# arhix52/Strelka

Hardware: AMD Instinct MI355X
Metric: Mray/s (higher is better)
Workload: dtype f32; 1 GPU; kitchen stand-in (SURVEY 8d C3): 1724134 unique triangles, 2022 instances of 153 meshes, 4 rect + 1 distant light, 60/25/10/5 % diffuse/glossy/metal/glass; resolution=1920x1080, bounces=4, spp=64, tile=32, world_size=1, parallelism=single GPU, rays_per_frame=839862650

## Files before the change

strelka_amd/csrc/skh_kernels.h:

```cpp
#pragma once
#include "skh_bvh.h"
#include "skh_env.h"
#include "skh_emit.h"
#include "skh_blend.h"

namespace skh
{

struct DevInstance
{
    float w2o[12];
    int rootRef;
    uint32_t mask;
    uint32_t type;
    uint32_t pad;
};
struct HostInstance
{
    float o2w[12];
    uint32_t type, geom, material, light;
};

#define SKH_WORLD_CURVES 2
#define SKH_SEG_STRIDE 8
// ... 151 lines not shown
    unsigned long long wave[2][10];
    unsigned long long shade[8];
    unsigned int slowCount, slowPad;
    float slow[16][12];
    unsigned long long runHist[2][42], blockHist[2][42];
    unsigned long long cyc[2][10];
#endif
#ifdef SKH_TAIL_PROFILE
    unsigned long long launchT0[2], dryHist[2][64], exitHist[2][64], afterDryHist[2][64], dryLive[2][65], rayTicksAfterDry[2], waveTicksAfterDry[2];
#endif
};

SKH_DI uint32_t rank_below(unsigned long long mask)
{
    return __builtin_amdgcn_mbcnt_hi((uint32_t)(mask >> 32), __builtin_amdgcn_mbcnt_lo((uint32_t)mask, 0u));
}
SKH_DI uint32_t wave_max(uint32_t v)
{
#pragma unroll
    for (int off = 32; off >= 1; off >>= 1)
        v = max(v, (uint32_t)__shfl_xor(v, off));
    return v;
}

SKH_DI uint32_t wave_sum(uint32_t v)
{
#pragma unroll
    for (int off = 32; off >= 1; off >>= 1)
        v += __shfl_xor(v, off);
    return v;
}

#ifndef SKH_CURVE_MIN_WAVES
#define SKH_CURVE_MIN_WAVES 6
#endif
#ifndef SKH_WORLD_CURVE_ANYHIT_MIN_WAVES
#define SKH_WORLD_CURVE_ANYHIT_MIN_WAVES 6
#endif
#ifndef SKH_WORLD_CURVE_MIN_WAVES
#define SKH_WORLD_CURVE_MIN_WAVES 6
#endif
#ifndef SKH_ANYHIT_MIN_WAVES
#define SKH_ANYHIT_MIN_WAVES 7
#endif
#ifndef SKH_TRACE_MIN_WAVES
#define SKH_TRACE_MIN_WAVES 7
#endif
#ifndef SKH_MATERIALS_LDS
#define SKH_MATERIALS_LDS 64
#endif
#ifndef SKH_WORLD_ANYHIT_MIN_WAVES
#define SKH_WORLD_ANYHIT_MIN_WAVES 8
#endif
#ifndef SKH_WORLD_CLOSEST_MIN_WAVES
#define SKH_WORLD_CLOSEST_MIN_WAVES 8
#endif
#ifndef SKH_TRACE_ATTR
#define SKH_TRACE_ATTR
#endif
#ifndef SKH_TRI_COOP
#define SKH_TRI_COOP 1
#endif
#define SKH_FETCH_STRIDE 32
#define SKH_COUNT_STRIDE 32

SKH_DI uint32_t skh_opaque(uint32_t v)
{
    asm volatile("" : "+s"(v));
    return v;
}
struct LightBox
{
    float lo[3], hi[3];
};
#ifndef SKH_BEST_LDS
#define SKH_BEST_LDS 1
#endif
#ifndef SKH_SEGNODE
#define SKH_SEGNODE 0
#endif
#ifndef SKH_ANYHIT_FLAT_PUSH
#define SKH_ANYHIT_FLAT_PUSH 1
#endif
template <bool ANY_HIT, bool COUNT, bool CURVES, bool WORLD = false, bool SPLIT = false>
__global__ void __launch_bounds__(SKH_TRACE_BLOCK, CURVES ? (WORLD ? (ANY_HIT ? SKH_WORLD_CURVE_ANYHIT_MIN_WAVES : SKH_WORLD_CURVE_MIN_WAVES) : SKH_CURVE_MIN_WAVES) : (WORLD ? (ANY_HIT ? SKH_WORLD_ANYHIT_MIN_WAVES : SKH_WORLD_CLOSEST_MIN_WAVES) : (ANY_HIT ? SKH_ANYHIT_MIN_WAVES : SKH_TRACE_MIN_WAVES))) SKH_TRACE_ATTR
    k_trace(DevScene sc, RayQ rq, const uint32_t* __restrict__ countPtr, uint32_t* __restrict__ fetch ,
            uint32_t fetchArg ,
            HitQ hq, PathS ps, const float4* __restrict__ contrib , int* __restrict__ ovfBase,
            StatsDev* __restrict__ stats, LightBox lightBox , uint32_t fetchChunk )
{
    constexpr bool TRICOOP = SKH_TRI_COOP && WORLD && !CURVES;
    constexpr bool BESTLDS = CURVES && !ANY_HIT && SKH_BEST_LDS;
    static_assert(!SPLIT || (WORLD && !CURVES), "SPLIT: the world-only triangle builds");
    constexpr int NLDS0 = (TRICOOP || BESTLDS) ? SKH_STACK_LDS - 1 : SKH_STACK_LDS;
    constexpr int NLDST = (SPLIT && NLDS0 >= 11) ? NLDS0 - 7 : NLDS0;
    static_assert(NLDS0 - NLDST <= SKH_TAIL_EXTRA, "the overflow columns' extra slots hold the LDS entries the tail phase gives up");
    __shared__ int s_stack[NLDS0 * SKH_TRACE_BLOCK];
    __shared__ uint32_t s_famx[(SPLIT && NLDST == NLDS0) ? 7 * SKH_TRACE_BLOCK : 1];
    uint32_t* const s_fam = NLDST < NLDS0 ? reinterpret_cast<uint32_t*>(s_stack + NLDST * SKH_TRACE_BLOCK) : s_famx;
    __shared__ uint32_t s_best[BESTLDS ? 4 * SKH_TRACE_BLOCK : 1];
    __shared__ unsigned char s_tab[(TRICOOP || SPLIT) ? 128 : 1];
    const uint32_t fetchMin = fetchArg & 0xffu, curveMin = (fetchArg >> 8) & 0xffu, nodeBreak = (fetchArg >> 16) & 0xffu, leafMin = fetchArg >> 24;
    const uint32_t lane = threadIdx.x;
    uint32_t n = 0;
#pragma unroll
    for (uint32_t g = 0; g < SKH_SHARDS; ++g)
        n += countPtr[g * SKH_COUNT_STRIDE];
    if (n == 0)
        return;
    const uint32_t perGroup = rq.region;
    const uint32_t group = blockIdx.x & 7u;
    uint32_t tries = 0;
    bool exhausted = false;
    uint32_t resBase = 0, resLeft = 0;
    uint32_t fam = threadIdx.x;
#define SKH_FAM(k, l) s_fam[(k) * SKH_TRACE_BLOCK + (l)]
    int* lds = s_stack + lane;
#define SKH_OVF_SLOT(e) ((SKH_TAIL_PHASE && (e) < NLDS0) ? SKH_STACK_OVF + ((e) - NLDSP) : (e) - NLDS0)
#define SKH_OVF_AT(e) ovfBase[(size_t)(e) * ovfStride + (skh_opaque(blockIdx.x * SKH_TRACE_BLOCK) + threadIdx.x)]
    const uint32_t ovfStride = gridDim.x * SKH_TRACE_BLOCK;
    const uint32_t rayMask = CURVES ? (ANY_HIT ? 3u : 255u) : (ANY_HIT ? 1u : 253u);
    TraceCounters tc = { 0, 0, 0, 0 };
#ifdef SKH_LANE_PROFILE
    uint32_t wv[10] = { 0, 0, 0, 0, 0, 0, 0, 0, 0, 0 };
    uint32_t rayNodes = 0, rayTris = 0, rayInsts = 0;
    unsigned long long cy[7] = { 0, 0, 0, 0, 0, 0, 0 };
    const unsigned long long cyStart = __builtin_readcyclecounter();
    const unsigned long long rtStart = __builtin_amdgcn_s_memrealtime();
#define SKH_LP(...) __VA_ARGS__
#else
#define SKH_LP(...)
#endif
#ifdef SKH_TAIL_PROFILE
    if (threadIdx.x == 0)
        atomicMin(&stats->launchT0[ANY_HIT ? 1 : 0], (unsigned long long)__builtin_amdgcn_s_memrealtime());
    bool dryNoted = false;
    unsigned long long dryLast = 0, dryAt = 0, rayTicks = 0;
    uint32_t dryLiveLanes = 0;
#endif

    bool hasRay = false, pending = false;
    uint32_t pend = 0;
    uint32_t ridx = 0;
    v3 ow = mk3(0.0f), dw = mk3(0.0f), o = mk3(0.0f), d = mk3(0.0f), inv = mk3(0.0f);
    v3 invw = mk3(0.0f);
    float tmin = 0.0f;
    RayShear sh;
    sh.perm = 0;
    sh.Sx = sh.Sy = sh.Sz = 0.0f;
    const Node4* nodes = sc.tlasNodes;
    bool inBlas = false;
    uint32_t curInst = 0, curType = 0;
    int sp = 0, cur = SKH_REF_INVALID;
    HitRec best;
    best.t = 0.0f, best.inst = best.prim = 0xffffffffu, best.u = best.v = 0.0f, best.found = false;

#define SKH_BEST_INST() (BESTLDS ? s_best[lane] : best.inst)
#define SKH_BEST_PRIM() (BESTLDS ? s_best[SKH_TRACE_BLOCK + lane] : best.prim)
#define SKH_BEST_SET(INST, PRIM, U, V)                                                                \
    {                                                                                                 \
        if (BESTLDS)                                                                                  \
        {                                                                                             \
            s_best[lane] = (INST), s_best[SKH_TRACE_BLOCK + lane] = (PRIM);                           \
            s_best[2 * SKH_TRACE_BLOCK + lane] = __float_as_uint(U), s_best[3 * SKH_TRACE_BLOCK + lane] = __float_as_uint(V); \
        }                                                                                             \
        else                                                                                          \
            best.inst = (INST), best.prim = (PRIM), best.u = (U), best.v = (V);                       \
    }
#define SKH_HIDDEN_LIGHT(C) (ANY_HIT && __float_as_uint((C).w) != 0u)
#define SKH_PUSH(v)                                                  \
    {                                                                \
        if (sp < NLDSP)                                              \
            lds[sp * SKH_TRACE_BLOCK] = (v);                         \
        else if (sp < NLDS0 + SKH_STACK_OVF)                         \
            SKH_OVF_AT(SKH_OVF_SLOT(sp)) = (v);                      \
        else                                                         \
            *sc.overflowFlag = 1u;  \
        ++sp;                                                        \
    }
#define SKH_POP(dst)                                                 \
    {                                                                \
        --sp;                                                        \
        if (sp < NLDSP)                                              \
            dst = lds[sp * SKH_TRACE_BLOCK];                         \
        else if (sp < NLDS0 + SKH_STACK_OVF)                         \
            dst = SKH_OVF_AT(SKH_OVF_SLOT(sp));                      \
        else                                                         \
            dst = SKH_REF_INVALID;                                   \
    }

#define SKH_CYLINDER_TESTS(FIRST, COUNT, PEND)                                                                                   \
    for (uint32_t k_ = 0; k_ < (COUNT); ++k_)                                                                                    \
// ... 9 lines not shown
    }
#define SKH_TAKE_MARKER()                                                                                         \
    {                                                                                                             \
        const uint32_t k = (uint32_t)cur & 0xffffu;                                                               \
        const uint32_t xinst = sc.worldCurveInst[k];           \
        curInst = ((sc.worldCurveMerged >> k) & 1u) ? 0xffffffffu : xinst;  \
        if ((uint32_t)cur & SKH_REF_CURVEROOT_IDENT)                                                              \
        {                                                                                                         \
             \
             \
            const float ident[12] = { 1.0f, 0.0f, 0.0f, 0.0f, 0.0f, 1.0f, 0.0f, 0.0f, 0.0f, 0.0f, 1.0f, 0.0f };    \
            o = xform_point_rel(ident, o);                                                                        \
            d = xform_vector(ident, d);                                                                           \
        }                                                                                                         \
        else                                                                                                      \
        {                                                                                                         \
            const float4* ip = reinterpret_cast<const float4*>(sc.inst + xinst);                                  \
            const float4 i0 = ip[0], i1 = ip[1], i2 = ip[2];                                                      \
            const v3 wo = mk3(rq.plane(0)[ridx], rq.plane(1)[ridx], rq.plane(2)[ridx]);                           \
            const v3 wd = mk3(rq.plane(3)[ridx], rq.plane(4)[ridx], rq.plane(5)[ridx]);                           \
            const float m[12] = { i0.x, i0.y, i0.z, i0.w, i1.x, i1.y, i1.z, i1.w, i2.x, i2.y, i2.z, i2.w };       \
            o = xform_point_rel(m, wo);                                                                           \
            d = xform_vector(m, wd);                                                                              \
        }                                                                                                         \
        inv = rcp3(d);                                                                                            \
        curType = 2;                                                                                              \
        cur = sc.worldCurveRoot[k];                                                                               \
    }

    {
        constexpr int NLDSP = NLDS0;
        constexpr bool TRICOOPP = TRICOOP;
#define SKH_TAIL_PHASE 0
        for (;;)
        {
#include "skh_trace_body.inc"
        }
#undef SKH_TAIL_PHASE
    }
    if constexpr (SPLIT)
    {
        constexpr int NLDSP = NLDST;
#ifndef SKH_TAIL_TRICOOP
#define SKH_TAIL_TRICOOP 1
#endif
        constexpr bool TRICOOPP = TRICOOP && SKH_TAIL_TRICOOP;
        if (NLDST < NLDS0)
        {
            for (int e = NLDST; e < NLDS0; ++e)
                if (hasRay && e < sp)
                    SKH_OVF_AT(SKH_STACK_OVF + e - NLDST) = lds[e * SKH_TRACE_BLOCK];
            __builtin_amdgcn_fence(__ATOMIC_RELEASE, "wavefront");
            __builtin_amdgcn_wave_barrier();
            __builtin_amdgcn_fence(__ATOMIC_ACQUIRE, "wavefront");
        }
        if (hasRay)
        {
            fam = lane;
            SKH_FAM(0, lane) = __float_as_uint(best.t);
            SKH_FAM(1, lane) = __float_as_uint(best.t);
            SKH_FAM(2, lane) = best.found ? (ANY_HIT ? 0u : best.inst) : 0xffffffffu;
            if constexpr (!ANY_HIT)
                SKH_FAM(3, lane) = best.prim, SKH_FAM(4, lane) = __float_as_uint(best.u), SKH_FAM(5, lane) = __float_as_uint(best.v);
            SKH_FAM(6, lane) = 1u;
        }
        __builtin_amdgcn_fence(__ATOMIC_RELEASE, "wavefront");
        __builtin_amdgcn_wave_barrier();
        __builtin_amdgcn_fence(__ATOMIC_ACQUIRE, "wavefront");
#define SKH_TAIL_PHASE 1
        for (;;)
        {
#include "skh_trace_body.inc"
        }
#undef SKH_TAIL_PHASE
    }
#undef SKH_PUSH
#undef SKH_HIDDEN_LIGHT
#undef SKH_POP
#undef SKH_OVF_AT
#undef SKH_OVF_SLOT
#undef SKH_TAKE_MARKER
#undef SKH_CYLINDER_TESTS
#undef SKH_FAM
#ifdef SKH_TAIL_PROFILE
    if (lane == 0 && dryNoted)
    {
        const int A = ANY_HIT ? 1 : 0;
        const unsigned long long t0 = *(volatile unsigned long long*)&stats->launchT0[A], now = __builtin_amdgcn_s_memrealtime();
        atomicAdd(&stats->dryHist[A][min(63ull, (dryAt - t0) / 1600ull)], 1ull);
        atomicAdd(&stats->exitHist[A][min(63ull, (now - t0) / 1600ull)], 1ull);
        atomicAdd(&stats->afterDryHist[A][min(63ull, (now - dryAt) / 1600ull)], 1ull);
        atomicAdd(&stats->dryLive[A][dryLiveLanes], 1ull);
        atomicAdd(&stats->rayTicksAfterDry[A], rayTicks);
        atomicAdd(&stats->waveTicksAfterDry[A], now - dryAt);
    }
#endif
    if (COUNT)
    {
        const uint32_t a = wave_sum(tc.nodes), b = wave_sum(tc.prims), c2 = wave_sum(tc.segs), d2 = wave_sum(tc.insts);
#ifdef SKH_LANE_PROFILE
        cy[5] = __builtin_readcyclecounter() - cyStart;
        if (lane == 0)
        {
            atomicAdd(&stats->cyc[ANY_HIT ? 1 : 0][6], cy[5]);
            atomicAdd(&stats->cyc[ANY_HIT ? 1 : 0][7], __builtin_amdgcn_s_memrealtime() - rtStart);
        }
        for (int k = 0; k < 7; ++k)
        {
            uint32_t hi = wave_max((uint32_t)(cy[k] >> 8));
            if (lane == 0)
                atomicAdd(&stats->cyc[ANY_HIT ? 1 : 0][k == 6 ? 8 : k], (unsigned long long)hi << 8);
        }
#endif
        if (lane == 0)
        {
            atomicAdd(&stats->nodes[ANY_HIT ? 1 : 0], (unsigned long long)a);
            atomicAdd(&stats->prims[ANY_HIT ? 1 : 0], (unsigned long long)b);
            atomicAdd(&stats->segs[ANY_HIT ? 1 : 0], (unsigned long long)c2);
            atomicAdd(&stats->insts[ANY_HIT ? 1 : 0], (unsigned long long)d2);
#ifdef SKH_LANE_PROFILE
            for (int k = 0; k < 10; ++k)
                atomicAdd(&stats->wave[ANY_HIT ? 1 : 0][k], (unsigned long long)wv[k]);
#endif
        }
    }
#undef SKH_LP
}

__global__ void k_hair_consts(const Material* __restrict__ mats, uint32_t n, HairConst* __restrict__ out)
{
    const uint32_t i = blockIdx.x * blockDim.x + threadIdx.x;
    if (i < n)
        out[i] = hair_const(mats[i]);
}

SKH_DI bool slot_to_pixel(const FrameP& fp, const uint32_t* __restrict__ tileXY, uint32_t slot, uint32_t& px, uint32_t& py)
{
    const uint32_t tile = slot >> (2 * fp.tileShift);
    const uint32_t m = slot & ((1u << (2 * fp.tileShift)) - 1u);
    px = tileXY[2 * tile] + compact1by1(m);
    py = tileXY[2 * tile + 1] + compact1by1(m >> 1);
    return px < fp.width && py < fp.height;
}

#define SKH_COMPACT_MAX_WAVES 8
SKH_DI uint32_t block_compact(bool emit, uint32_t* counter, uint32_t* s_wave )
{
    const uint32_t lane = threadIdx.x & 63u, wave = threadIdx.x >> 6, nw = blockDim.x >> 6;
    const unsigned long long m = __ballot(emit);
    if (lane == 0)
        s_wave[wave] = (uint32_t)__popcll(m);
    __syncthreads();
    if (threadIdx.x == 0)
    {
        uint32_t tot = 0;
        for (uint32_t w = 0; w < nw; ++w)
        {
            const uint32_t cnt = s_wave[w];
            s_wave[w] = tot;
            tot += cnt;
        }
        s_wave[SKH_COMPACT_MAX_WAVES] = tot ? atomicAdd(counter, tot) : 0u;
    }
    __syncthreads();
    const uint32_t r = s_wave[SKH_COMPACT_MAX_WAVES] + s_wave[wave] + rank_below(m);
    __syncthreads();
// ... 1044 lines not shown
```

strelka_amd/csrc/skh_shade_body.inc:

```
    const uint32_t numPick = (ENV ? sc.numLights + (env.nee ? 1u : 0u) : sc.numLights) + (EMIT ? (emit.nee ? 1u : 0u) : 0u);
    __shared__ uint32_t s_wave[2 * (SKH_COMPACT_MAX_WAVES + 1)];
    __shared__ uint32_t s_sobol[SKH_SOBOL_LUT_WORDS];
#if SKH_MATERIALS_LDS
    __shared__ float4 s_mat[SKH_MATERIALS_LDS * 4];
#endif
    const uint32_t shard = blockIdx.x & (SKH_SHARDS - 1u), lb = blockIdx.x / SKH_SHARDS;
    const uint32_t n = countPtr[shard * SKH_COUNT_STRIDE];
    if (lb * blockDim.x >= n)
        return;
    const uint32_t il = lb * blockDim.x + threadIdx.x;
    const uint32_t i = shard * rq.region + il;
#ifdef SKH_LANE_PROFILE
    unsigned long long spc[8] = { 0, 0, 0, 0, 0, 0, 0, 0 }, spT = __builtin_readcyclecounter();
#define SKH_SP(k)                                                    \
    {                                                                \
        const unsigned long long t_ = __builtin_readcyclecounter();  \
        spc[k] += t_ - spT;                                          \
        spT = t_;                                                    \
    }
#else
#define SKH_SP(k)
#endif
    bool valid = il < n;
    uint32_t pid = 0;
    v3 rayO = mk3(0.0f), rayD = mk3(0.0f);
    float4 hr0 = make_float4(0.0f, 0.0f, 0.0f, 0.0f), hr1 = hr0;
    {
        constexpr int passes = ((SKH_SOBOL_LUT_WORDS / 4) + SKH_SHADE_BLOCK - 1) / SKH_SHADE_BLOCK;
        uint4 lut[passes];
#pragma unroll
        for (int k = 0; k < passes; ++k)
            if ((k + 1) * SKH_SHADE_BLOCK <= SKH_SOBOL_LUT_WORDS / 4 || threadIdx.x + k * SKH_SHADE_BLOCK < SKH_SOBOL_LUT_WORDS / 4)
                lut[k] = reinterpret_cast<const uint4*>(g_sobol_lut)[threadIdx.x + k * SKH_SHADE_BLOCK];
            else
                lut[k] = make_uint4(0u, 0u, 0u, 0u);
#if SKH_MATERIALS_LDS
        float4 mrow = make_float4(0.0f, 0.0f, 0.0f, 0.0f);
        static_assert(SKH_MATERIALS_LDS * 4 <= SKH_SHADE_BLOCK, "one float4 of the material table per thread");
        if (threadIdx.x < SKH_MATERIALS_LDS * 4 && threadIdx.x < sc.numMaterials * 4u)
            mrow = reinterpret_cast<const float4*>(sc.materials)[threadIdx.x];
#endif
#pragma unroll
        for (int k = 0; k < passes; ++k)
            if ((k + 1) * SKH_SHADE_BLOCK <= SKH_SOBOL_LUT_WORDS / 4 || threadIdx.x + k * SKH_SHADE_BLOCK < SKH_SOBOL_LUT_WORDS / 4)
                reinterpret_cast<uint4*>(s_sobol)[threadIdx.x + k * SKH_SHADE_BLOCK] = lut[k];
#if SKH_MATERIALS_LDS
        if (threadIdx.x < SKH_MATERIALS_LDS * 4)
            s_mat[threadIdx.x] = mrow;
#endif
    }
    __syncthreads();
    bool emitNext = false, emitShadow = false;
    v3 nextO = mk3(0.0f), nextD = mk3(0.0f), shO = mk3(0.0f), shD = mk3(0.0f), shC = mk3(0.0f);
    float shTmax = 0.0f;
    if (valid)
    {
        pid = rq.ids()[i];
        rayO = mk3(rq.plane(0)[i], rq.plane(1)[i], rq.plane(2)[i]);
        rayD = mk3(rq.plane(3)[i], rq.plane(4)[i], rq.plane(5)[i]);
        if (hq.primBits != 0u)
        {
            hr0 = *hq.rec16(i);
            const uint32_t w = __float_as_uint(hr0.w);
            hr1.x = __uint_as_float(w == 0xffffffffu ? w : w >> hq.primBits);
            hr1.y = __uint_as_float(w == 0xffffffffu ? w : ((w & ((1u << hq.primBits) - 1u)) | (hq.direct ? SKH_PRIM_DIRECT : 0u)));
        }
        else
            hr0 = hq.rec(i)[0], hr1 = hq.rec(i)[1];
        const float ht = hr0.x, hu = hr0.y, hv = hr0.z;
        const uint32_t hinst = __float_as_uint(hr1.x), hprim = __float_as_uint(hr1.y);
        float* P = ps.base;
        const size_t S = ps.stride;
        v3 throughput = depth == 0u ? mk3(1.0f) : mk3(P[pid], P[pid + S], P[pid + 2 * S]);
        v3 radiance = mk3(0.0f);
        bool radianceDirty = false;
#define SKH_RADIANCE_LOAD() radiance = mk3(ps.rad()[pid]), radianceDirty = true
        float lastBsdfPdf = depth == 0u ? 0.0f : P[pid + 6 * S];
        uint32_t flags = depth == 0u ? 0u : reinterpret_cast<uint32_t*>(P)[pid + 7 * S];
        bool inside = (flags & PF_INSIDE) != 0;
        bool specularBounce = (flags & PF_SPECULAR) != 0;
        uint32_t firstEvent = (flags >> PF_EVENT_SHIFT) & 3u;
        uint32_t px, py;
        const uint32_t sub = pid / fp.numSlots;
        slot_to_pixel(fp, tileXY, pid - sub * fp.numSlots, px, py);
        Sampler smp = init_sampler(px, py, fp.subframeIndex + sampleOffset + sub, fp.sppTotal, 52u);
        smp.depth = depth;
        uint32_t prdDepth = depth;
        v3 origin = rayO, dir = rayD;

        if (hinst == 0xffffffffu)
        {
            if constexpr (ENV)
            {
                const EnvEval ee = env_eval(env, rayD);
                SKH_RADIANCE_LOAD();
                if (depth == 0 || specularBounce || !env.nee)
                    radiance = radiance + throughput * ee.Le;
                else
                {
                    const float lightPdf = ee.pdf / (float)numPick;
                    const float misWeight = mis_weight_balance(lastBsdfPdf, lightPdf);
                    radiance = radiance + throughput * ee.Le * misWeight;
                }
            }
            else
            {
                const v3 bg = throughput * mk3(0.0f);
                if (!(bg.x == 0.0f && bg.y == 0.0f && bg.z == 0.0f))
                {
                    SKH_RADIANCE_LOAD();
                    radiance = radiance + bg;
                }
            }
            throughput = mk3(0.0f);
            prdDepth = fp.maxDepth;
        }
        else
        {
            SKH_SP(0)
            const HostInstance hi = sc.instances[hinst];
            const float* w2o = sc.inst[hinst].w2o;
            const bool directTv = (hprim & SKH_PRIM_DIRECT) != 0u;
            float4 tv[3], tx[2];
            const bool txWanted = HAIR || sc.numTextures != 0u;
            tx[0] = tx[1] = make_float4(0.0f, 0.0f, 0.0f, 0.0f);
            {
                const uint32_t recIdx = directTv ? (hprim & ~SKH_PRIM_DIRECT) : 0u;
                const float4* tp = sc.shadeTris + 6 * (size_t)(hq.primBits ? min(recIdx, hq.recClamp) : recIdx);
#pragma unroll
                for (int k = 0; k < 3; ++k)
                    tv[k] = tp[k];
                if (txWanted)
                    tx[0] = tp[3], tx[1] = tp[4];
            }
            asm volatile("" ::"v"(hi.type), "v"(hi.material), "v"(hi.light));
            if (hi.type == 1)
            {
                const uint32_t lidx = hi.light < sc.numLights ? hi.light : 0u;
                const Light& l = sc.lights[lidx];
                const v3 hitPoint = rayO + ht * rayD;
                if constexpr (LSHAPE)
                {
                    const Lshape lse = lshape_fetch(lsh, lidx);
                    const bool sampledDisc = l.type == 1 && (lse.flags & SKH_LSHAPE_SAMPLE_DISC) != 0u;
                    const v3 lightNormal = sampledDisc ? normalize(mk3(l.normal)) : calc_light_normal(l, hitPoint);
                    if (-dot(rayD, lightNormal) > 0.0f)
                    {
                        const v3 Li = mk3(l.color) * lshape_cone(lse, -rayD);
                        SKH_RADIANCE_LOAD();
                        if (depth == 0 || specularBounce)
                            radiance = radiance + throughput * Li * -dot(rayD, lightNormal);
                        else
                        {
                            const float lightPdf = (sampledDisc ? disc_light_pdf(l, hitPoint, rayO) : get_light_pdf(l, hitPoint, rayO)) / (float)numPick;
                            const float misWeight = mis_weight_balance(lastBsdfPdf, lightPdf);
                            radiance = radiance + throughput * Li * -dot(rayD, lightNormal) * misWeight;
                        }
                    }
                }
                else
                {
                    const v3 lightNormal = calc_light_normal(l, hitPoint);
                    if (-dot(rayD, lightNormal) > 0.0f)
                    {
                        SKH_RADIANCE_LOAD();
                        if (depth == 0 || specularBounce)
                            radiance = radiance + throughput * mk3(l.color) * -dot(rayD, lightNormal);
                        else
                        {
                            const float lightPdf = get_light_pdf(l, hitPoint, rayO) / (float)numPick;
                            const float misWeight = mis_weight_balance(lastBsdfPdf, lightPdf);
                            radiance = radiance + throughput * mk3(l.color) * -dot(rayD, lightNormal) * misWeight;
                        }
                    }
                }
                throughput = mk3(0.0f);
            }
            else
            {
                const uint32_t mid = hi.material == 0xffffffffu ? 0u : hi.material;
                float4 matLe = make_float4(0.0f, 0.0f, 0.0f, 0.0f);
                if constexpr (EMIT)
                    matLe = emit.Le[mid < emit.numMaterials ? mid : 0u];
                MtexEntry mte;
                if constexpr (MTEX)
                    mte = mtex_entry(mtex, mid < sc.numMaterials ? mid : 0u);
#if SKH_MATERIALS_LDS
                const uint32_t midc = mid < sc.numMaterials ? mid : 0u;
                Material mat;
                if (midc < (uint32_t)SKH_MATERIALS_LDS)
                {
                    const float4 m0 = s_mat[4 * midc], m1 = s_mat[4 * midc + 1], m2 = s_mat[4 * midc + 2], m3 = s_mat[4 * midc + 3];
                    mat.type = __float_as_uint(m0.x), mat.base_color[0] = m0.y, mat.base_color[1] = m0.z, mat.base_color[2] = m0.w;
                    mat.roughness = m1.x, mat.metallic = m1.y, mat.specular = m1.z, mat.ior = m1.w;
                    mat.base_color_texture = __float_as_uint(m2.x), mat.normal_texture = __float_as_uint(m2.y);
                    mat.reserved[0] = m2.z, mat.reserved[1] = m2.w, mat.reserved[2] = m3.x, mat.reserved[3] = m3.y, mat.reserved[4] = m3.z, mat.reserved[5] = m3.w;
                }
                else
                    mat = sc.materials[midc];
#else
                Material mat = sc.materials[mid < sc.numMaterials ? mid : 0u];
#endif
                if (!directTv && hi.type != 2)
                {
                    const float4* tp = sc.shadeTris + 6 * (size_t)(hi.light + hprim);
#pragma unroll
                    for (int k = 0; k < 3; ++k)
                        tv[k] = tp[k];
                    if (txWanted)
                        tx[0] = tp[3], tx[1] = tp[4];
                }
                asm volatile("" ::"v"(mat.type), "v"(tv[0].x), "v"(tv[1].x), "v"(tv[2].x));
                const bool useBase = mat.base_color_texture != 0u && mat.base_color_texture <= sc.numTextures;
                const bool useNormal = mat.normal_texture != 0u && mat.normal_texture <= sc.numTextures;
                bool mtexWanted = false;
                if constexpr (MTEX)
                    mtexWanted = mtex_wanted(mat, mte, sc.numTextures, matLe.w > 0.0f);
// ... 319 lines not shown
```

strelka_amd/csrc/skh_trace_body.inc:

```
        const unsigned long long needMask = __ballot(!hasRay);
        const uint32_t want = (uint32_t)__popcll(needMask);
        SKH_LP(wv[3]++; unsigned long long cyA = __builtin_readcyclecounter();)
#ifdef SKH_TAIL_PROFILE
        if (exhausted)
        {
            const unsigned long long now = __builtin_amdgcn_s_memrealtime();
            if (!dryNoted)
                dryNoted = true, dryAt = now, dryLiveLanes = 64u - want;
            else
                rayTicks += (unsigned long long)(64u - want) * (now - dryLast);
            dryLast = now;
        }
#endif
        if (want >= fetchMin || want == 64u || SKH_TAIL_PHASE)
        {
            if (pending)
            {
                pending = false;
                const uint32_t i = ridx;
                if (ANY_HIT)
                {
                    if (hq.base)
                        hq.base[i] = best.found ? 1.0f : -1.0f;
                    else if (!best.found)
                    {
                        const float4 cw = contrib[i];
                        float4* rad = ps.rad() + __float_as_uint(cw.w);
                        float4 r = *rad;
                        r.x += cw.x;
                        r.y += cw.y;
                        r.z += cw.z;
                        *rad = r;
                    }
                }
                else
                {
                    float4* hr = hq.rec(i);
                    if (BESTLDS && hq.primBits != 0u)
                    {
                        const bool f = best.found;
                        *hq.rec16(i) = make_float4(f ? best.t : -1.0f, f ? __uint_as_float(s_best[2 * SKH_TRACE_BLOCK + lane]) : 0.0f, f ? __uint_as_float(s_best[3 * SKH_TRACE_BLOCK + lane]) : 0.0f,
                                                   __uint_as_float(f ? (s_best[lane] << hq.primBits) | (s_best[SKH_TRACE_BLOCK + lane] & ((1u << hq.primBits) - 1u)) : 0xffffffffu));
                    }
                    else if (BESTLDS)
                    {
                        const bool f = best.found;
                        hr[0] = make_float4(f ? best.t : -1.0f, f ? __uint_as_float(s_best[2 * SKH_TRACE_BLOCK + lane]) : 0.0f,
                                            f ? __uint_as_float(s_best[3 * SKH_TRACE_BLOCK + lane]) : 0.0f, 0.0f);
                        hr[1] = make_float4(__uint_as_float(f ? s_best[lane] : 0xffffffffu), __uint_as_float(f ? s_best[SKH_TRACE_BLOCK + lane] : 0xffffffffu), 0.0f, 0.0f);
                    }
                    else if (hq.primBits != 0u)
                        *hq.rec16(i) = make_float4(best.found ? best.t : -1.0f, best.u, best.v,
                                                   __uint_as_float(best.found ? (best.inst << hq.primBits) | (best.prim & ((1u << hq.primBits) - 1u)) : 0xffffffffu));
                    else
                    {
                        hr[0] = make_float4(best.found ? best.t : -1.0f, best.u, best.v, 0.0f);
                        hr[1] = make_float4(__uint_as_float(best.inst), __uint_as_float(best.prim), 0.0f, 0.0f);
                    }
                }
            }
        }
#if !SKH_TAIL_PHASE
        if (!exhausted && (want >= fetchMin || want == 64u))
        {
            SKH_LP(wv[4]++; wv[5] += want;)
            uint32_t base = 0, count = 0, base2 = 0, count1 = 0;
            if constexpr (WORLD && !CURVES)
            {
                const uint32_t chunk = fetchChunk;
                count1 = min(want, resLeft);
                base = resBase, count = count1;
                resBase += count1, resLeft -= count1;
                if (count1 < want)
                {
                    const uint32_t ask = chunk ? chunk : want;
                    const int leader = __ffsll((long long)needMask) - 1;
                    while (tries < 8u)
                    {
                        const uint32_t g = (group + tries) & 7u;
                        uint32_t b = 0;
                        if ((int)lane == leader)
                            b = atomicAdd(&fetch[g * SKH_FETCH_STRIDE], ask);
                        b = (uint32_t)__builtin_amdgcn_readlane((int)b, leader);
                        const uint32_t lo = g * perGroup;
                        const uint32_t hi = lo + min(countPtr[g * SKH_COUNT_STRIDE], perGroup);
                        if (lo < hi && b < hi - lo)
                        {
                            const uint32_t got = min(ask, hi - (lo + b));
                            if (got < ask)
                                ++tries;
                            const uint32_t count2 = min(want - count1, got);
                            base2 = lo + b;
                            if (chunk)
                                resBase = base2 + count2, resLeft = got - count2;
                            count = count1 + count2;
                            break;
                        }
                        ++tries;
                    }
                    if (tries >= 8u && count == 0)
                        exhausted = true;
                }
            }
            else
            {
                const int leader = __ffsll((long long)needMask) - 1;
                while (tries < 8u)
                {
                    const uint32_t g = (group + tries) & 7u;
                    uint32_t b = 0;
                    if ((int)lane == leader)
                        b = atomicAdd(&fetch[g * SKH_FETCH_STRIDE], want);
                    b = __shfl(b, leader);
                    const uint32_t lo = g * perGroup;
                    const uint32_t hi = lo + min(countPtr[g * SKH_COUNT_STRIDE], perGroup);
                    if (lo < hi && b < hi - lo)
                    {
                        base = lo + b;
                        count = min(want, hi - base);
                        if (count < want)
                            ++tries;
                        break;
                    }
                    ++tries;
                }
                if (tries >= 8u && count == 0)
                    exhausted = true;
            }
            const uint32_t rank = rank_below(needMask);
            if (!hasRay && rank < count)
            {
                ridx = (WORLD && !CURVES) ? (rank < count1 ? base + rank : base2 + (rank - count1)) : base + rank;
                ow = mk3(rq.plane(0)[ridx], rq.plane(1)[ridx], rq.plane(2)[ridx]);
                dw = mk3(rq.plane(3)[ridx], rq.plane(4)[ridx], rq.plane(5)[ridx]);
                tmin = rq.plane(6)[ridx];
                o = ow;
                d = dw;
                inv = rcp3(d);
                if (ANY_HIT && !WORLD)
                    invw = inv;
                const int wr0 = sc.worldRoot;
                int wr1 = ANY_HIT ? SKH_REF_INVALID : sc.lightRoot;
                if (!ANY_HIT && wr1 != SKH_REF_INVALID)
                {
                    const float lnx = ((inv.x >= 0.0f ? lightBox.lo[0] : lightBox.hi[0]) - o.x) * inv.x, lfx = ((inv.x >= 0.0f ? lightBox.hi[0] : lightBox.lo[0]) - o.x) * inv.x;
                    const float lny = ((inv.y >= 0.0f ? lightBox.lo[1] : lightBox.hi[1]) - o.y) * inv.y, lfy = ((inv.y >= 0.0f ? lightBox.hi[1] : lightBox.lo[1]) - o.y) * inv.y;
                    const float lnz = ((inv.z >= 0.0f ? lightBox.lo[2] : lightBox.hi[2]) - o.z) * inv.z, lfz = ((inv.z >= 0.0f ? lightBox.hi[2] : lightBox.lo[2]) - o.z) * inv.z;
                    const float ltn = fmaxf(fmaxf(lnx, lny), fmaxf(lnz, tmin)), ltf = fminf(fminf(lfx, lfy), fminf(lfz, rq.plane(7)[ridx] ));
                    if (!(ltn <= ltf * SKH_SLAB_SLACK))
                        wr1 = SKH_REF_INVALID;
                }
                if (WORLD && CURVES)
                {
                    if (!CURVES)
                        sh = make_shear(dw);
                    curInst = 0xffffffffu;
                    curType = 0;
                    sp = 0;
                    for (uint32_t k = 0; k < sc.numWorldCurves; ++k)
                        SKH_PUSH((int)(SKH_REF_CURVEROOT | k | ((k + 1u == sc.numWorldCurves && sc.worldCurveIdentLast) ? SKH_REF_CURVEROOT_IDENT : 0u)))
                    if (wr0 != SKH_REF_INVALID && wr1 != SKH_REF_INVALID)
                        SKH_PUSH(wr1)
                    cur = wr0 != SKH_REF_INVALID ? wr0 : wr1;
                    if (cur == SKH_REF_INVALID)
                        SKH_POP(cur)
                }
                else if (wr0 != SKH_REF_INVALID || wr1 != SKH_REF_INVALID)
                {
                    if (!CURVES)
                        sh = make_shear(dw);
                    nodes = sc.triNodes;
                    inBlas = true;
                    curInst = 0xffffffffu;
                    curType = 0;
                    sp = 0;
                    if (!WORLD && sc.tlasRoot != SKH_REF_INVALID)
                    {
                        lds[0] = sc.tlasRoot;
                        lds[SKH_TRACE_BLOCK] = SKH_REF_SENTINEL;
                        sp = 2;
                    }
                    if (wr0 != SKH_REF_INVALID && wr1 != SKH_REF_INVALID)
                        lds[(sp++) * SKH_TRACE_BLOCK] = wr1;
                    cur = wr0 != SKH_REF_INVALID ? wr0 : wr1;
                }
                else
                {
                    nodes = sc.tlasNodes;
                    inBlas = false;
                    sp = 0;
                    cur = sc.tlasRoot;
                }
                best.t = rq.plane(7)[ridx];
                best.inst = best.prim = 0xffffffffu;
                best.u = best.v = 0.0f;
                best.found = false;
                pend = 0;
                hasRay = true;
            }
        }
        if (SPLIT && exhausted)
            break;
#else
        {
            {
                if (!ANY_HIT && hasRay && best.found)
                    atomicMin(&SKH_FAM(0, fam), __float_as_uint(best.t));
                __builtin_amdgcn_fence(__ATOMIC_RELEASE, "wavefront");
                __builtin_amdgcn_wave_barrier();
                __builtin_amdgcn_fence(__ATOMIC_ACQUIRE, "wavefront");
                bool famDone = false;
                if (hasRay)
                {
                    if (ANY_HIT)
                    {
                        if (SKH_FAM(2, fam) != 0xffffffffu)
                        {
                            famDone = true;
                            best.found = true;
                            cur = SKH_REF_INVALID;
                            sp = 0;
                        }
                    }
                    else
                    {
                        const uint32_t tb = SKH_FAM(0, fam);
                        if (__uint_as_float(tb) < best.t)
                        {
                            best.t = __uint_as_float(tb + 1u);
                            best.found = false;
                            best.inst = best.prim = 0xffffffffu;
                            best.u = best.v = 0.0f;
                        }
                    }
                }
                const bool giver = hasRay && sp > 0 && !famDone;
                const unsigned long long idleM = __ballot(!hasRay), giveM = __ballot(giver);
                const uint32_t nI = (uint32_t)__popcll(idleM), nG = (uint32_t)__popcll(giveM);
                if (nI != 0u && nG != 0u)
                {
                    const uint32_t rI = rank_below(idleM), rG = rank_below(giveM);
                    if (giver)
                        s_tab[rG] = (unsigned char)lane;
                    __builtin_amdgcn_fence(__ATOMIC_RELEASE, "wavefront");
                    __builtin_amdgcn_wave_barrier();
                    __builtin_amdgcn_fence(__ATOMIC_ACQUIRE, "wavefront");
                    const bool idle = !hasRay;
                    const int depth = idle ? (int)(rI / nG) : 0;
                    const int src = idle ? (int)s_tab[rI % nG] : (int)lane;
                    const int psp = __shfl(sp, src);
                    const bool takes = idle && depth < psp && depth < NLDS0 + SKH_STACK_OVF;
                    int pgive = SKH_REF_INVALID;
                    if (takes)
                    {
                        const int e = min(psp, NLDS0 + SKH_STACK_OVF) - 1 - depth;
                        pgive = e < NLDSP ? s_stack[e * SKH_TRACE_BLOCK + src] : ovfBase[(size_t)SKH_OVF_SLOT(e) * ovfStride + (blockIdx.x * SKH_TRACE_BLOCK + (uint32_t)src)];
                    }
                    if (giver)
                    {
                        const uint32_t offered = nI > rG ? (nI - rG + nG - 1u) / nG : 0u;
                        const uint32_t gone = min(min((uint32_t)sp, (uint32_t)(NLDS0 + SKH_STACK_OVF)), offered);
                        if (gone != 0u)
                        {
                            atomicAdd(&SKH_FAM(6, fam), gone);
                            sp = min(sp, NLDS0 + SKH_STACK_OVF) - (int)gone;
                        }
                    }
#define SKH_TAKE_F(X)                      \
    {                                      \
        const float t_ = __shfl((X), src); \
        if (takes)                         \
            (X) = t_;                      \
    }
#define SKH_TAKE_U(X)                                      \
    {                                                      \
        const uint32_t t_ = (uint32_t)__shfl((int)(X), src); \
        if (takes)                                         \
            (X) = t_;                                      \
    }
                    SKH_TAKE_F(o.x) SKH_TAKE_F(o.y) SKH_TAKE_F(o.z)
                    SKH_TAKE_F(inv.x) SKH_TAKE_F(inv.y) SKH_TAKE_F(inv.z)
                    SKH_TAKE_F(sh.Sx) SKH_TAKE_F(sh.Sy) SKH_TAKE_F(sh.Sz)
                    {
// ... 675 lines not shown
```

Measured before the change: 6193 Mray/s.

## Interleave ray refill with result writeback and hoist shade loads for latency overlap

Merges the trace kernel's result-writeback block and the work-queue refill block into one section. The any-hit contribution load and the radiance read-modify-write now straddle the refill's atomic and ray loads, and the per-shard counts are loaded once into registers instead of re-read from memory on each refill. In the shade kernel, the instance record and triangle shading-data loads are hoisted ahead of flag and sampler setup, and pixel coordinates are computed inline, so the memory latency overlaps with other work. Empty asm barriers pin the load ordering, at the cost of more live registers and possible occupancy loss.

Result: no change. 6230 Mray/s, median of 6 (+0.6%).

```diff
diff --git a/strelka_amd/csrc/skh_kernels.h b/strelka_amd/csrc/skh_kernels.h
--- a/strelka_amd/csrc/skh_kernels.h
+++ b/strelka_amd/csrc/skh_kernels.h
@@ -257,6 +257,9 @@
 #ifndef SKH_ANYHIT_FLAT_PUSH
 #define SKH_ANYHIT_FLAT_PUSH 1
 #endif
+#ifndef SKH_ANYHIT_EARLY_CONTRIB
+#define SKH_ANYHIT_EARLY_CONTRIB 1
+#endif
 template <bool ANY_HIT, bool COUNT, bool CURVES, bool WORLD = false, bool SPLIT = false>
 __global__ void __launch_bounds__(SKH_TRACE_BLOCK, CURVES ? (WORLD ? (ANY_HIT ? SKH_WORLD_CURVE_ANYHIT_MIN_WAVES : SKH_WORLD_CURVE_MIN_WAVES) : SKH_CURVE_MIN_WAVES) : (WORLD ? (ANY_HIT ? SKH_WORLD_ANYHIT_MIN_WAVES : SKH_WORLD_CLOSEST_MIN_WAVES) : (ANY_HIT ? SKH_ANYHIT_MIN_WAVES : SKH_TRACE_MIN_WAVES))) SKH_TRACE_ATTR
     k_trace(DevScene sc, RayQ rq, const uint32_t* __restrict__ countPtr, uint32_t* __restrict__ fetch ,
@@ -277,12 +280,13 @@
     __shared__ unsigned char s_tab[(TRICOOP || SPLIT) ? 128 : 1];
     const uint32_t fetchMin = fetchArg & 0xffu, curveMin = (fetchArg >> 8) & 0xffu, nodeBreak = (fetchArg >> 16) & 0xffu, leafMin = fetchArg >> 24;
     const uint32_t lane = threadIdx.x;
-    uint32_t n = 0;
-#pragma unroll
-    for (uint32_t g = 0; g < SKH_SHARDS; ++g)
-        n += countPtr[g * SKH_COUNT_STRIDE];
-    if (n == 0)
-        return;
+    static_assert(SKH_SHARDS == 8, "the refill walks eight shards");
+    const uint32_t shardLen0 = countPtr[0], shardLen1 = countPtr[SKH_COUNT_STRIDE], shardLen2 = countPtr[2 * SKH_COUNT_STRIDE], shardLen3 = countPtr[3 * SKH_COUNT_STRIDE];
+    const uint32_t shardLen4 = countPtr[4 * SKH_COUNT_STRIDE], shardLen5 = countPtr[5 * SKH_COUNT_STRIDE], shardLen6 = countPtr[6 * SKH_COUNT_STRIDE], shardLen7 = countPtr[7 * SKH_COUNT_STRIDE];
+    if (shardLen0 + shardLen1 + shardLen2 + shardLen3 + shardLen4 + shardLen5 + shardLen6 + shardLen7 == 0u)
+        return;
+#define SKH_SHARD_LEN(g) \
+    ((g) == 0u ? shardLen0 : (g) == 1u ? shardLen1 : (g) == 2u ? shardLen2 : (g) == 3u ? shardLen3 : (g) == 4u ? shardLen4 : (g) == 5u ? shardLen5 : (g) == 6u ? shardLen6 : shardLen7)
     const uint32_t perGroup = rq.region;
     const uint32_t group = blockIdx.x & 7u;
     uint32_t tries = 0;
@@ -458,6 +462,7 @@
 #undef SKH_TAKE_MARKER
 #undef SKH_CYLINDER_TESTS
 #undef SKH_FAM
+#undef SKH_SHARD_LEN
 #ifdef SKH_TAIL_PROFILE
     if (lane == 0 && dryNoted)
     {
diff --git a/strelka_amd/csrc/skh_shade_body.inc b/strelka_amd/csrc/skh_shade_body.inc
--- a/strelka_amd/csrc/skh_shade_body.inc
+++ b/strelka_amd/csrc/skh_shade_body.inc
@@ -61,12 +61,16 @@
         if (hq.primBits != 0u)
         {
             hr0 = *hq.rec16(i);
+            asm volatile("" ::"v"(hr0.x), "v"(hr0.y), "v"(hr0.z), "v"(hr0.w));
             const uint32_t w = __float_as_uint(hr0.w);
             hr1.x = __uint_as_float(w == 0xffffffffu ? w : w >> hq.primBits);
             hr1.y = __uint_as_float(w == 0xffffffffu ? w : ((w & ((1u << hq.primBits) - 1u)) | (hq.direct ? SKH_PRIM_DIRECT : 0u)));
         }
         else
+        {
             hr0 = hq.rec(i)[0], hr1 = hq.rec(i)[1];
+            asm volatile("" ::"v"(hr0.x), "v"(hr0.y), "v"(hr0.z), "v"(hr1.x), "v"(hr1.y));
+        }
         const float ht = hr0.x, hu = hr0.y, hv = hr0.z;
         const uint32_t hinst = __float_as_uint(hr1.x), hprim = __float_as_uint(hr1.y);
         float* P = ps.base;
@@ -77,12 +81,31 @@
 #define SKH_RADIANCE_LOAD() radiance = mk3(ps.rad()[pid]), radianceDirty = true
         float lastBsdfPdf = depth == 0u ? 0.0f : P[pid + 6 * S];
         uint32_t flags = depth == 0u ? 0u : reinterpret_cast<uint32_t*>(P)[pid + 7 * S];
+        const uint32_t sub = pid / fp.numSlots;
+        const uint32_t slot = pid - sub * fp.numSlots, tile = slot >> (2 * fp.tileShift);
+        const uint32_t tileX = tileXY[2 * tile], tileY = tileXY[2 * tile + 1];
+        HostInstance hi;
+        float4 tv[3], tx[2];
+        const bool directTv = (hprim & SKH_PRIM_DIRECT) != 0u;
+        const bool txWanted = HAIR || sc.numTextures != 0u;
+        tx[0] = tx[1] = make_float4(0.0f, 0.0f, 0.0f, 0.0f);
+        if (hinst != 0xffffffffu)
+        {
+            hi = sc.instances[hinst];
+            const uint32_t recIdx = directTv ? (hprim & ~SKH_PRIM_DIRECT) : 0u;
+            const float4* tp = sc.shadeTris + 6 * (size_t)(hq.primBits ? min(recIdx, hq.recClamp) : recIdx);
+#pragma unroll
+            for (int k = 0; k < 3; ++k)
+                tv[k] = tp[k];
+            if (txWanted)
+                tx[0] = tp[3], tx[1] = tp[4];
+        }
+        asm volatile("" ::: "memory");
         bool inside = (flags & PF_INSIDE) != 0;
         bool specularBounce = (flags & PF_SPECULAR) != 0;
         uint32_t firstEvent = (flags >> PF_EVENT_SHIFT) & 3u;
-        uint32_t px, py;
-        const uint32_t sub = pid / fp.numSlots;
-        slot_to_pixel(fp, tileXY, pid - sub * fp.numSlots, px, py);
+        const uint32_t slotM = slot & ((1u << (2 * fp.tileShift)) - 1u);
+        const uint32_t px = tileX + compact1by1(slotM), py = tileY + compact1by1(slotM >> 1);
         Sampler smp = init_sampler(px, py, fp.subframeIndex + sampleOffset + sub, fp.sppTotal, 52u);
         smp.depth = depth;
         uint32_t prdDepth = depth;
@@ -118,21 +141,7 @@
         else
         {
             SKH_SP(0)
-            const HostInstance hi = sc.instances[hinst];
             const float* w2o = sc.inst[hinst].w2o;
-            const bool directTv = (hprim & SKH_PRIM_DIRECT) != 0u;
-            float4 tv[3], tx[2];
-            const bool txWanted = HAIR || sc.numTextures != 0u;
-            tx[0] = tx[1] = make_float4(0.0f, 0.0f, 0.0f, 0.0f);
-            {
-                const uint32_t recIdx = directTv ? (hprim & ~SKH_PRIM_DIRECT) : 0u;
-                const float4* tp = sc.shadeTris + 6 * (size_t)(hq.primBits ? min(recIdx, hq.recClamp) : recIdx);
-#pragma unroll
-                for (int k = 0; k < 3; ++k)
-                    tv[k] = tp[k];
-                if (txWanted)
-                    tx[0] = tp[3], tx[1] = tp[4];
-            }
             asm volatile("" ::"v"(hi.type), "v"(hi.material), "v"(hi.light));
             if (hi.type == 1)
             {
diff --git a/strelka_amd/csrc/skh_trace_body.inc b/strelka_amd/csrc/skh_trace_body.inc
--- a/strelka_amd/csrc/skh_trace_body.inc
+++ b/strelka_amd/csrc/skh_trace_body.inc
@@ -12,8 +12,93 @@
             dryLast = now;
         }
 #endif
-        if (want >= fetchMin || want == 64u || SKH_TAIL_PHASE)
+        const bool writeNow = want >= fetchMin || want == 64u || SKH_TAIL_PHASE;
+#if SKH_TAIL_PHASE
+        constexpr bool refill = false;
+#else
+        const bool refill = !exhausted && writeNow;
+#endif
+        if (writeNow)
         {
+            float4 cw = make_float4(0.0f, 0.0f, 0.0f, 0.0f), radv = cw;
+            float* rad = nullptr;
+            bool addRad = false;
+            if (SKH_ANYHIT_EARLY_CONTRIB && ANY_HIT && pending && !hq.base && !best.found)
+            {
+                cw = contrib[ridx];
+                addRad = true;
+            }
+            uint32_t base = 0, count = 0, base2 = 0, count1 = 0;
+#if !SKH_TAIL_PHASE
+            if (refill)
+            {
+                SKH_LP(wv[4]++; wv[5] += want;)
+                if constexpr (WORLD && !CURVES)
+                {
+                    const uint32_t chunk = fetchChunk;
+                    count1 = min(want, resLeft);
+                    base = resBase, count = count1;
+                    resBase += count1, resLeft -= count1;
+                    if (count1 < want)
+                    {
+                        const uint32_t ask = chunk ? chunk : want;
+                        const int leader = __ffsll((long long)needMask) - 1;
+                        while (tries < 8u)
+                        {
+                            const uint32_t g = (group + tries) & 7u;
+                            uint32_t b = 0;
+                            if ((int)lane == leader)
+                                b = atomicAdd(&fetch[g * SKH_FETCH_STRIDE], ask);
+                            b = (uint32_t)__builtin_amdgcn_readlane((int)b, leader);
+                            const uint32_t lo = g * perGroup;
+                            const uint32_t hi = lo + min(SKH_SHARD_LEN(g), perGroup);
+                            if (lo < hi && b < hi - lo)
+                            {
+                                const uint32_t got = min(ask, hi - (lo + b));
+                                if (got < ask)
+                                    ++tries;
+                                const uint32_t count2 = min(want - count1, got);
+                                base2 = lo + b;
+                                if (chunk)
+                                    resBase = base2 + count2, resLeft = got - count2;
+                                count = count1 + count2;
+                                break;
+                            }
+                            ++tries;
+                        }
+                        if (tries >= 8u && count == 0)
+                            exhausted = true;
+                    }
+                }
+                else
+                {
+                    const int leader = __ffsll((long long)needMask) - 1;
+                    while (tries < 8u)
+                    {
+                        const uint32_t g = (group + tries) & 7u;
+                        uint32_t b = 0;
+                        if ((int)lane == leader)
+                            b = atomicAdd(&fetch[g * SKH_FETCH_STRIDE], want);
+                        b = __shfl(b, leader);
+                        const uint32_t lo = g * perGroup;
+                        const uint32_t hi = lo + min(SKH_SHARD_LEN(g), perGroup);
+                        if (lo < hi && b < hi - lo)
+                        {
+                            base = lo + b;
+                            count = min(want, hi - base);
+                            if (count < want)
+                                ++tries;
+                            break;
+                        }
+                        ++tries;
+                    }
+                    if (tries >= 8u && count == 0)
+                        exhausted = true;
+                }
+            }
+#endif
+            if (SKH_ANYHIT_EARLY_CONTRIB && ANY_HIT)
+                asm volatile("" ::"v"(cw.x), "v"(cw.y), "v"(cw.z), "v"(cw.w));
             if (pending)
             {
                 pending = false;
@@ -22,15 +107,14 @@
                 {
                     if (hq.base)
                         hq.base[i] = best.found ? 1.0f : -1.0f;
-                    else if (!best.found)
-                    {
-                        const float4 cw = contrib[i];
-                        float4* rad = ps.rad() + __float_as_uint(cw.w);
-                        float4 r = *rad;
-                        r.x += cw.x;
-                        r.y += cw.y;
-                        r.z += cw.z;
-                        *rad = r;
+                    else if (SKH_ANYHIT_EARLY_CONTRIB ? addRad : !best.found)
+                    {
+                        if (!SKH_ANYHIT_EARLY_CONTRIB)
+                            cw = contrib[i], addRad = true;
+                        uint32_t path = __float_as_uint(cw.w);
+                        asm volatile("" : "+v"(path));
+                        rad = &(ps.rad() + path)->x;
+                        radv.x = rad[0], radv.y = rad[1], radv.z = rad[2];
                     }
                 }
                 else
@@ -59,146 +143,93 @@
                     }
                 }
             }
+#if !SKH_TAIL_PHASE
+            if (refill)
+            {
+                const uint32_t rank = rank_below(needMask);
+                if (!hasRay && rank < count)
+                {
+                    ridx = (WORLD && !CURVES) ? (rank < count1 ? base + rank : base2 + (rank - count1)) : base + rank;
+                    ow = mk3(rq.plane(0)[ridx], rq.plane(1)[ridx], rq.plane(2)[ridx]);
+                    dw = mk3(rq.plane(3)[ridx], rq.plane(4)[ridx], rq.plane(5)[ridx]);
+                    tmin = rq.plane(6)[ridx];
+                    const float tmax = rq.plane(7)[ridx];
+                    o = ow;
+                    d = dw;
+                    inv = rcp3(d);
+                    if (ANY_HIT && !WORLD)
+                        invw = inv;
+                    const int wr0 = sc.worldRoot;
+                    int wr1 = ANY_HIT ? SKH_REF_INVALID : sc.lightRoot;
+                    if (!ANY_HIT && wr1 != SKH_REF_INVALID)
+                    {
+                        const float lnx = ((inv.x >= 0.0f ? lightBox.lo[0] : lightBox.hi[0]) - o.x) * inv.x, lfx = ((inv.x >= 0.0f ? lightBox.hi[0] : lightBox.lo[0]) - o.x) * inv.x;
+                        const float lny = ((inv.y >= 0.0f ? lightBox.lo[1] : lightBox.hi[1]) - o.y) * inv.y, lfy = ((inv.y >= 0.0f ? lightBox.hi[1] : lightBox.lo[1]) - o.y) * inv.y;
+                        const float lnz = ((inv.z >= 0.0f ? lightBox.lo[2] : lightBox.hi[2]) - o.z) * inv.z, lfz = ((inv.z >= 0.0f ? lightBox.hi[2] : lightBox.lo[2]) - o.z) * inv.z;
+                        const float ltn = fmaxf(fmaxf(lnx, lny), fmaxf(lnz, tmin)), ltf = fminf(fminf(lfx, lfy), fminf(lfz, tmax));
+                        if (!(ltn <= ltf * SKH_SLAB_SLACK))
+                            wr1 = SKH_REF_INVALID;
+                    }
+                    if (WORLD && CURVES)
+                    {
+                        if (!CURVES)
+                            sh = make_shear(dw);
+                        curInst = 0xffffffffu;
+                        curType = 0;
+                        sp = 0;
+                        for (uint32_t k = 0; k < sc.numWorldCurves; ++k)
+                            SKH_PUSH((int)(SKH_REF_CURVEROOT | k | ((k + 1u == sc.numWorldCurves && sc.worldCurveIdentLast) ? SKH_REF_CURVEROOT_IDENT : 0u)))
+                        if (wr0 != SKH_REF_INVALID && wr1 != SKH_REF_INVALID)
+                            SKH_PUSH(wr1)
+                        cur = wr0 != SKH_REF_INVALID ? wr0 : wr1;
+                        if (cur == SKH_REF_INVALID)
+                            SKH_POP(cur)
+                    }
+                    else if (wr0 != SKH_REF_INVALID || wr1 != SKH_REF_INVALID)
+                    {
+                        if (!CURVES)
+                            sh = make_shear(dw);
+                        nodes = sc.triNodes;
+                        inBlas = true;
+                        curInst = 0xffffffffu;
+                        curType = 0;
+                        sp = 0;
+                        if (!WORLD && sc.tlasRoot != SKH_REF_INVALID)
+                        {
+                            lds[0] = sc.tlasRoot;
+                            lds[SKH_TRACE_BLOCK] = SKH_REF_SENTINEL;
+                            sp = 2;
+                        }
+                        if (wr0 != SKH_REF_INVALID && wr1 != SKH_REF_INVALID)
+                            lds[(sp++) * SKH_TRACE_BLOCK] = wr1;
+                        cur = wr0 != SKH_REF_INVALID ? wr0 : wr1;
+                    }
+                    else
+                    {
+                        nodes = sc.tlasNodes;
+                        inBlas = false;
+                        sp = 0;
+                        cur = sc.tlasRoot;
+                    }
+                    best.t = tmax;
+                    best.inst = best.prim = 0xffffffffu;
+                    best.u = best.v = 0.0f;
+                    best.found = false;
+                    pend = 0;
+                    hasRay = true;
+                }
+            }
+#endif
+            if (ANY_HIT)
+                asm volatile("" ::"v"(radv.x), "v"(radv.y), "v"(radv.z));
+            if (ANY_HIT && addRad)
+            {
+                rad[0] = radv.x + cw.x;
+                rad[1] = radv.y + cw.y;
+                rad[2] = radv.z + cw.z;
+            }
         }
 #if !SKH_TAIL_PHASE
-        if (!exhausted && (want >= fetchMin || want == 64u))
-        {
-            SKH_LP(wv[4]++; wv[5] += want;)
-            uint32_t base = 0, count = 0, base2 = 0, count1 = 0;
-            if constexpr (WORLD && !CURVES)
-            {
-                const uint32_t chunk = fetchChunk;
-                count1 = min(want, resLeft);
-                base = resBase, count = count1;
-                resBase += count1, resLeft -= count1;
-                if (count1 < want)
-                {
-                    const uint32_t ask = chunk ? chunk : want;
-                    const int leader = __ffsll((long long)needMask) - 1;
-                    while (tries < 8u)
-                    {
-                        const uint32_t g = (group + tries) & 7u;
-                        uint32_t b = 0;
-                        if ((int)lane == leader)
-                            b = atomicAdd(&fetch[g * SKH_FETCH_STRIDE], ask);
-                        b = (uint32_t)__builtin_amdgcn_readlane((int)b, leader);
-                        const uint32_t lo = g * perGroup;
-                        const uint32_t hi = lo + min(countPtr[g * SKH_COUNT_STRIDE], perGroup);
-                        if (lo < hi && b < hi - lo)
-                        {
-                            const uint32_t got = min(ask, hi - (lo + b));
-                            if (got < ask)
-                                ++tries;
-                            const uint32_t count2 = min(want - count1, got);
-                            base2 = lo + b;
-                            if (chunk)
-                                resBase = base2 + count2, resLeft = got - count2;
-                            count = count1 + count2;
-                            break;
-                        }
-                        ++tries;
-                    }
-                    if (tries >= 8u && count == 0)
-                        exhausted = true;
-                }
-            }
-            else
-            {
-                const int leader = __ffsll((long long)needMask) - 1;
-                while (tries < 8u)
-                {
-                    const uint32_t g = (group + tries) & 7u;
-                    uint32_t b = 0;
-                    if ((int)lane == leader)
-                        b = atomicAdd(&fetch[g * SKH_FETCH_STRIDE], want);
-                    b = __shfl(b, leader);
-                    const uint32_t lo = g * perGroup;
-                    const uint32_t hi = lo + min(countPtr[g * SKH_COUNT_STRIDE], perGroup);
-                    if (lo < hi && b < hi - lo)
-                    {
-                        base = lo + b;
-                        count = min(want, hi - base);
-                        if (count < want)
-                            ++tries;
-                        break;
-                    }
-                    ++tries;
-                }
-                if (tries >= 8u && count == 0)
-                    exhausted = true;
-            }
-            const uint32_t rank = rank_below(needMask);
-            if (!hasRay && rank < count)
-            {
-                ridx = (WORLD && !CURVES) ? (rank < count1 ? base + rank : base2 + (rank - count1)) : base + rank;
-                ow = mk3(rq.plane(0)[ridx], rq.plane(1)[ridx], rq.plane(2)[ridx]);
-                dw = mk3(rq.plane(3)[ridx], rq.plane(4)[ridx], rq.plane(5)[ridx]);
-                tmin = rq.plane(6)[ridx];
-                o = ow;
-                d = dw;
-                inv = rcp3(d);
-                if (ANY_HIT && !WORLD)
-                    invw = inv;
-                const int wr0 = sc.worldRoot;
-                int wr1 = ANY_HIT ? SKH_REF_INVALID : sc.lightRoot;
-                if (!ANY_HIT && wr1 != SKH_REF_INVALID)
-                {
-                    const float lnx = ((inv.x >= 0.0f ? lightBox.lo[0] : lightBox.hi[0]) - o.x) * inv.x, lfx = ((inv.x >= 0.0f ? lightBox.hi[0] : lightBox.lo[0]) - o.x) * inv.x;
-                    const float lny = ((inv.y >= 0.0f ? lightBox.lo[1] : lightBox.hi[1]) - o.y) * inv.y, lfy = ((inv.y >= 0.0f ? lightBox.hi[1] : lightBox.lo[1]) - o.y) * inv.y;
-                    const float lnz = ((inv.z >= 0.0f ? lightBox.lo[2] : lightBox.hi[2]) - o.z) * inv.z, lfz = ((inv.z >= 0.0f ? lightBox.hi[2] : lightBox.lo[2]) - o.z) * inv.z;
-                    const float ltn = fmaxf(fmaxf(lnx, lny), fmaxf(lnz, tmin)), ltf = fminf(fminf(lfx, lfy), fminf(lfz, rq.plane(7)[ridx] ));
-                    if (!(ltn <= ltf * SKH_SLAB_SLACK))
-                        wr1 = SKH_REF_INVALID;
-                }
-                if (WORLD && CURVES)
-                {
-                    if (!CURVES)
-                        sh = make_shear(dw);
-                    curInst = 0xffffffffu;
-                    curType = 0;
-                    sp = 0;
-                    for (uint32_t k = 0; k < sc.numWorldCurves; ++k)
-                        SKH_PUSH((int)(SKH_REF_CURVEROOT | k | ((k + 1u == sc.numWorldCurves && sc.worldCurveIdentLast) ? SKH_REF_CURVEROOT_IDENT : 0u)))
-                    if (wr0 != SKH_REF_INVALID && wr1 != SKH_REF_INVALID)
-                        SKH_PUSH(wr1)
-                    cur = wr0 != SKH_REF_INVALID ? wr0 : wr1;
-                    if (cur == SKH_REF_INVALID)
-                        SKH_POP(cur)
-                }
-                else if (wr0 != SKH_REF_INVALID || wr1 != SKH_REF_INVALID)
-                {
-                    if (!CURVES)
-                        sh = make_shear(dw);
-                    nodes = sc.triNodes;
-                    inBlas = true;
-                    curInst = 0xffffffffu;
-                    curType = 0;
-                    sp = 0;
-                    if (!WORLD && sc.tlasRoot != SKH_REF_INVALID)
-                    {
-                        lds[0] = sc.tlasRoot;
-                        lds[SKH_TRACE_BLOCK] = SKH_REF_SENTINEL;
-                        sp = 2;
-                    }
-                    if (wr0 != SKH_REF_INVALID && wr1 != SKH_REF_INVALID)
-                        lds[(sp++) * SKH_TRACE_BLOCK] = wr1;
-                    cur = wr0 != SKH_REF_INVALID ? wr0 : wr1;
-                }
-                else
-                {
-                    nodes = sc.tlasNodes;
-                    inBlas = false;
-                    sp = 0;
-                    cur = sc.tlasRoot;
-                }
-                best.t = rq.plane(7)[ridx];
-                best.inst = best.prim = 0xffffffffu;
-                best.u = best.v = 0.0f;
-                best.found = false;
-                pend = 0;
-                hasRay = true;
-            }
-        }
         if (SPLIT && exhausted)
             break;
 #else
```
